# aouyang1/go-muse

Measured on AMD Instinct MI355X. Metric: series-pairs XCorr/sec at N=4096, 1M-series batch; achieved HBM GB/s, higher is better.
Workload: dtype f64

## Files before the change

### go-muse_amd/binding.py

```python
import ctypes
import os

import numpy as np

from . import build as _build

_i32 = ctypes.c_int32
_i64 = ctypes.c_int64
_f64 = ctypes.c_double
_vp = ctypes.c_void_p
_dp = ctypes.POINTER(ctypes.c_double)
_i32p = ctypes.POINTER(ctypes.c_int32)
_i64p = ctypes.POINTER(ctypes.c_int64)

MUSE_OK = 0
MUSE_ERR_INVALID = -1
MUSE_ERR_LENGTH = -2
MUSE_ERR_ZERO_STD = -3
MUSE_ERR_NO_DEVICE = -4
MUSE_ERR_HIP = -5
MUSE_ERR_UNSUPPORTED = -6
MUSE_ERR_NOMEM = -7
MUSE_ERR_EMPTY = -8
MUSE_LAG_WINDOW_MAX = 63
# ... 117 lines not shown
    "muse_test_many_lag_range_plan": (ctypes.c_int, [_i32, _i32, _i32, _i32, _i32, _i32p]),
    "muse_test_window_many_plan_rows": (ctypes.c_int, [_i32, _i32, _i32p, _i32p, _i32p, _i32p, _i32p, _i32p]),
    "muse_batch_run_many": (ctypes.c_int, [ctypes.POINTER(_vp), _i32, _i32p, _i32, _i32, _i32, _f64, _i32, _i32,
                                           _i64p, _i32p, _dp, _i32p, _dp]),
    "muse_batch_free": (ctypes.c_int, [_vp]),
    "muse_xcorr_with_x": (ctypes.c_int, [_vp, _dp, _dp, _i32, _i32, _dp, _i32p, _dp, _i32p]),
    "muse_xcorr": (ctypes.c_int, [_vp, _dp, _i32, _dp, _i32, _i32, _i32, _dp, _i32p, _dp, _i32p]),
    "muse_xcorr_groups": (ctypes.c_int, [_vp, _vp, _i32, _i32, _i32p, _dp, _i32p, _dp]),
    "muse_xcorr_batch": (ctypes.c_int, [_vp, _dp, _dp, _i64, _i32, _i32, _i32, _i32, _i32p, _dp, _i32p, _dp]),
    "muse_ctx_set_spectrum_cache": (ctypes.c_int, [_vp, _i32]),
    "muse_group_spectrum_cache": (ctypes.c_int, [_vp, _i64p, _i64p]),
    "muse_group_drop_spectrum_cache": (ctypes.c_int, [_vp]),
    "muse_test_spectrum_cache_limits": (ctypes.c_int, [_vp, _i64, _i64]),
    "muse_test_spectrum_cache_reader": (ctypes.c_int, [_vp, _i32]),
    "muse_test_spectrum_cache_policy": (ctypes.c_int, [_i64, _i32, _i32, _i32, _i64, _i64, _i64, _i32p, _i64p, _i64p]),
    "muse_test_batch_redo_pairs": (ctypes.c_int, [_vp, _i64p, _i64, _i64p]),
    "muse_next_pow2": (_i64, [_f64]),
}


class MuseError(RuntimeError):
    def __init__(self, status, message):
        super().__init__("muse_hip status %d: %s" % (status, message))
        self.status = status
        self.message = message


_lib = None


# ... 45 lines not shown
```

### go-muse_amd/csrc/capi_batch.hip

```cpp
#include "capi_internal.h"
#include "xcorr_huge.h"

using namespace muse;


int ilog2(int64_t n)
{
    int l = 0;
    while (((int64_t)1 << l) < n)
        l++;
    return l;
}

int build_spectrum(muse_ctx *ctx, const double *ref_host, int N, int n, int normalize, double x_scale,
                          double xc_scale, double2 *X, double2 *xc, float2 *xcf, double *xs, int *zero_std)
{
    double *dref = nullptr;
    int *dstat = nullptr;
    double2 *dscr = nullptr;
    HIP_TRY(dmalloc(ctx, &dref, (size_t)N * sizeof(double)));
    hipError_t e = dmalloc(ctx, &dstat, sizeof(int));
    if (e == hipSuccess && n > GENERIC_LDS_MAX_N)
        e = dmalloc(ctx, &dscr, (size_t)n * sizeof(double2));
    if (e == hipSuccess)
// ... 335 lines not shown
        kc.variant = KERNEL_REAL_SPLIT;
        kc.gsmall = ctx->gsmall[4];
    } else if ((b->n == 32768 || (b->n == 65536 && (b->N == b->n || b->c1))) && (ctx->variant == 0 || ctx->variant == 14) && !b->g->f32 && ctx->gsmall[4]) {
        kc.variant = KERNEL_REAL;
        kc.gsmall = ctx->gsmall[4];
    } else if (b->xcp && has_twl && (b->N == b->n || b->c1) && ((b->n >= 32768 && ctx->variant == 0) || (b->n >= 16384 && ctx->variant == 13))) {
        kc.variant = KERNEL_LONG;
    } else if (((b->n >= 512 && b->n <= 2048) || b->n == 8192 || b->n == 16384) && (ctx->variant == 0 || ctx->variant == 12)) {
        kc.variant = KERNEL_SMALL;
    } else if (((b->n >= 512 && b->n <= 2048) || b->n >= 8192) && (ctx->variant == 0 || ctx->variant == 11)) {
        kc.variant = KERNEL_STOCKHAM;
    }
    return kc;
}

int spectrum_cache_policy(int64_t rows, int32_t N, bool f32, int mode, int64_t min_rows, int64_t free_bytes, int64_t budget,
                          int64_t *rows_cached, int64_t *bytes)
{
    *rows_cached = 0;
    *bytes = 0;
    if (mode != 1 || f32 || N <= 2048 || N > 4096 || rows < std::max<int64_t>(min_rows, 2))
        return ZC_POLICY_NONE;
    const int64_t pairs = rows / 2;
    *rows_cached = 2 * pairs;
    *bytes = pairs * ZC_PAIR_BYTES;
    const int64_t limit = budget >= 0 ? budget : free_bytes / 2;
    return *bytes <= limit ? ZC_POLICY_BUILD : ZC_POLICY_DECLINED;
}

void group_drop_spectrum_cache(muse_group *g)
// ... 141 lines not shown
    ctx->zc_reader.store(reader);
    return MUSE_OK;
}

extern "C" int muse_test_spectrum_cache_policy(int64_t rows, int32_t N, int32_t f32, int32_t mode, int64_t min_rows,
                                               int64_t free_bytes, int64_t budget_bytes, int32_t *decision,
                                               int64_t *rows_cached, int64_t *bytes)
{
    if (!decision || !rows_cached || !bytes)
        return fail(MUSE_ERR_INVALID, "NULL output");
    *decision = spectrum_cache_policy(rows, N, f32 != 0, mode, min_rows < 0 ? ZC_MIN_ROWS : min_rows, free_bytes,
                                      budget_bytes < 0 ? -1 : budget_bytes, rows_cached, bytes);
    return MUSE_OK;
}

extern "C" int muse_test_batch_redo_pairs(muse_batch *b, int64_t *pairs, int64_t cap, int64_t *count)
{
    if (!b || !count || cap < 0 || (cap > 0 && !pairs))
        return fail(MUSE_ERR_INVALID, "bad redo-list arguments");
    *count = 0;
    int rc = use_device(b->ctx);
    if (rc)
        return rc;
    HIP_TRY(hipStreamSynchronize(b->stream()));
    if (!b->ovf_count || !b->ovf_list.p)
        return MUSE_OK;
    int listed = 0;
    HIP_TRY(hipMemcpy(&listed, b->ovf_count, sizeof(int), hipMemcpyDeviceToHost));
    *count = listed;
    const int64_t k = std::min<int64_t>(std::min<int64_t>(listed, cap), b->ovf_list.cap);
// ... 11 lines not shown
{
    *variant = -1;
    if (win_L < 0 && b->windowed())
        return MUSE_OK;
    if (b->n > GENERIC_MAX_N)
        return b->g->f32 ? fail(MUSE_ERR_UNSUPPORTED, "float32-storage groups run on the default kernels only (FFT lengths 512 ... 16384)") : MUSE_OK;
    const KernelChoice kc = choose_kernel(b, (b->g->M + 1) / 2);
    if (kc.error)
        return fail(MUSE_ERR_UNSUPPORTED, "%s", kc.error);
    if (win_L >= 0 && (!(kc.variant == KERNEL_R16_FOLD || kc.variant == KERNEL_R16_OCC3 || (kc.variant == KERNEL_SMALL && b->logn <= 11)) || 2 * win_L > b->n))
        return fail(MUSE_ERR_UNSUPPORTED, "the masked transform pass runs on the default kernels of FFT lengths 512 ... 4096");
    *variant = kc.variant;
    return MUSE_OK;
}

int batch_score(muse_batch *b, bool allow_spectrum_cache, int win_L, const SlideFuse *slide, int win_lneg)
{
    if (!b)
        return fail(MUSE_ERR_INVALID, "NULL batch");
    muse_ctx *ctx = b->ctx;
    int rc = use_device(ctx);
    if (rc)
        return rc;
    rc = group_ready(b->g, b->stream());
    if (rc)
        return rc;
    const int64_t M = b->g->M;
    if (M == 0)
        return MUSE_OK;
    const hipStream_t st = b->stream();
    rc = ensure_scores(b);
    if (rc)
        return rc;
    b->origin = ScoreOrigin{};
    if (win_L < 0 && b->windowed()) {
        b->scores_exact = true;
        return score_windowed(b);
    }
    if (b->n > GENERIC_MAX_N) {
        if (b->g->f32)
            return fail(MUSE_ERR_UNSUPPORTED, "float32-storage groups run on the default kernels only (FFT lengths 512 ... 16384)");
        b->scores_exact = true;
        return huge_score(b);
    }
    std::unique_lock<std::mutex> scratch_lock(ctx->stage_mu, std::defer_lock);
    if (b->n >= GENERIC_LDS_MAX_N)
        scratch_lock.lock();
    FusedParams p = base_params(b);
    b->scores_exact = true;
// ... 15 lines not shown
            b->origin = ScoreOrigin::in_window(MUSE_IN_WINDOW_MASKED, win_L, variant);
            set_window(p, win_L);
        }
    }
    if (slide) {
        if (variant != KERNEL_R16_FOLD || allow_spectrum_cache)
            return fail(MUSE_ERR_INVALID, "the fused slide runs in the default n = 4096 kernel, off the rows");
        p.slide_tails = slide->tails;
        p.slide_k = slide->k;
    }
    if (variant == KERNEL_GENERIC && b->n <= GENERIC_LDS_MAX_N)
        p.gscratch = nullptr;
    LaunchTimer timer(ctx, false, st);
    LaunchTimer redo_timer(ctx, true, st);
    if (variant == KERNEL_R16_FOLD) {
        HIP_TRY(b->ovf_list.ensure(ctx, 2 * p.npairs, st));
        p.ovf_count = b->ovf_count;
        p.work_counter = b->ovf_count + 1;
        p.ovf_list = b->ovf_list.p;
        HIP_TRY(hipMemsetAsync(b->ovf_count, 0, 2 * sizeof(int), st));
        ZcPlan plan;
        std::unique_lock<std::mutex> zc_lock(b->g->ready_mu, std::defer_lock);
        if (allow_spectrum_cache && win_L < 0 && spectrum_cache_candidate(b, variant)) {
            zc_lock.lock();
            rc = plan_spectrum_cache(b, plan);
            if (rc)
                return rc;
            if (!plan.use)
                zc_lock.unlock();
        }
        HIP_TRY(timer.begin());
        if (plan.use) {
            bool launched = false;
            const auto next_launch = [&]() {
                const hipError_t e = launched ? hipMemsetAsync(b->ovf_count + 1, 0, sizeof(int), st) : hipSuccess;
// ... 15 lines not shown
                                                               plan.tail_zpairs ? plan.tail_seg.zstat() : nullptr,
                                                               plan.tail_pair0, plan.tail_zpairs}, ctx->num_cus, st));
            }
            zc_lock.unlock();
        } else {
            HIP_TRY(launch_fused(p, variant, ctx->num_cus, st));
        }
        HIP_TRY(timer.end());
        FusedParams q = p;
        q.slide_tails = nullptr;
        q.slide_k = 0;
        q.pair_list = b->ovf_list.p;
        q.pair_count = b->ovf_count;
        q.dense_total = ctx->variant == 0 ? p.npairs : 0;
        q.npairs = std::min<long long>(p.npairs, (long long)ctx->num_cus * 3);
        HIP_TRY(redo_timer.begin());
        HIP_TRY(launch_fused(q, KERNEL_R16_OCC3, ctx->num_cus, st));
        HIP_TRY(redo_timer.end());
        if (p.npairs >= 1024 && !(b->handoff_host && b->handoff_M == M && b->handoff_rewrites == b->g->rewrites)) {
            if (!b->handoff_host)
                HIP_TRY(hmalloc(ctx, &b->handoff_host, sizeof(int)));
            *b->handoff_host = 0;
            b->handoff_M = M;
            b->handoff_rewrites = b->g->rewrites;
            HIP_TRY(hipMemcpyAsync(b->handoff_host, b->ovf_count, sizeof(int), hipMemcpyDeviceToHost, st));
        }
    } else if (variant == KERNEL_LONG) {
        HIP_TRY(b->ovf_list.ensure(ctx, 2 * p.npairs, st));
        p.ovf_count = b->ovf_count;
        p.ovf_list = b->ovf_list.p;
        HIP_TRY(hipMemsetAsync(b->ovf_count, 0, 2 * sizeof(int), st));
        HIP_TRY(timer.begin());
        HIP_TRY(launch_fused(p, variant, ctx->num_cus, st));
// ... 152 lines not shown
```

### go-muse_amd/csrc/capi_internal.h

```cpp
#pragma once
#include <hip/hip_runtime.h>

#include <algorithm>
#include <atomic>
#include <mutex>
#include <cmath>
#include <cstdarg>
#include <cstdio>
#include <cstdlib>
#include <cstring>
#include <ctime>
#include <limits>
#include <map>
#include <new>
#include <string>
#include <unordered_map>
#include <utility>
#include <vector>

#include "muse_hip.h"
#include "muse_hip_test.h"
#include "xcorr_kernels.h"

using namespace muse;
// ... 92 lines not shown
    MemPool dev_pool, host_pool;
    HugeWork huge;
    int huge_batch_mb = 0;
    std::mutex huge_mu;
    std::mutex small_mu;
    std::vector<std::pair<unsigned char *, int>> small_free;
    unsigned long long small_token = 0;
    std::mutex timing_mu;
    std::atomic<bool> rows_always_copy{false};
    std::vector<void *> rows_slots;
    std::mutex rows_mu;
    std::atomic<int> zc_mode{1};
    std::atomic<int64_t> zc_min_rows{ZC_MIN_ROWS};
    std::atomic<int64_t> zc_budget{-1};
    std::atomic<int> zc_reader{0};
    std::atomic<int> win_rows_slices{0};
    std::atomic<bool> in_window_force{false};
    std::atomic<int> slide_in_window_force{0};
    std::atomic<bool> gather_nt{false};
    std::atomic<int> refs{1};
};

struct muse_group {
    std::atomic<int> refs{1};
    muse_ctx *ctx = nullptr;
    double *rows = nullptr;
    float *rows32 = nullptr;
    bool f32 = false;
    size_t elem() const { return f32 ? sizeof(float) : sizeof(double); }
    void *base() const { return f32 ? (void *)rows32 : (void *)rows; }
// ... 76 lines not shown

struct muse_batch {
    muse_ctx *ctx = nullptr;
    muse_group *g = nullptr;
    hipStream_t own_stream = nullptr;
    hipStream_t stream() const { return own_stream ? own_stream : ctx->stream; }
    int32_t N = 0, n = 0, logn = 0;
    muse_spectrum *sp = nullptr;
    double *c1 = nullptr;
    double2 *X = nullptr, *xc = nullptr;
    double2 *xcp = nullptr;
    double2 *xcw = nullptr;
    float2 *xcf = nullptr;
    double *xs = nullptr;
    int *ovf_count = nullptr;
    int *handoff_host = nullptr;
    int64_t handoff_M = -1;
    uint64_t handoff_rewrites = 0;
    PoolBuf<long long> ovf_list;
    PoolBuf<double> mv;
    PoolBuf<int> lag;
    unsigned char *small_out = nullptr;
    int small_cap = 0;
    PoolBuf<int> gid_dev;
    std::vector<int32_t> gid_host;
    bool gid_valid = false;
    PoolBuf<unsigned long long> gkey;
    PoolBuf<long long> gfirst, gwin;
    GroupWork gw() const { return GroupWork{gkey.p, gfirst.p, gwin.p}; }
    PoolBuf<muse_record> rec;
// ... 99 lines not shown
void huge_free(muse_ctx *ctx);
int huge_reference(muse_ctx *ctx, const double *ref_host, int N, int n, double2 *X, double2 *table, int *zero_std);
int huge_score(muse_batch *b);
int huge_pairs(muse_ctx *ctx, const double *xrows, int64_t xstride, int Nx, int normalize_x, double x_scale, const double *yrows,
               int64_t ystride, int Ny, int normalize_y, int64_t M, int n, double cc_scale, double *mv, int *lag, int *nil, double *cc);
void adopt_spectrum(muse_batch *b);
int build_spectrum(muse_ctx *ctx, const double *ref_host, int N, int n, int normalize, double x_scale,
                          double xc_scale, double2 *X, double2 *xc, float2 *xcf, double *xs, int *zero_std);
hipError_t ensure_gscratch(muse_ctx *ctx, int64_t n, int slices_per_cu = muse::GSCRATCH_SLICES_PER_CU);
hipError_t ensure_twl(muse_ctx *ctx, int64_t n);
int ensure_scores(muse_batch *b);
struct SlideFuse {
    const void *tails;
    int32_t k;
};
int batch_score(muse_batch *b, bool allow_spectrum_cache, int win_L = -1, const SlideFuse *slide = nullptr, int win_lneg = -1);
int batch_score_check(muse_batch *b, int win_L, int *variant);
enum { ZC_POLICY_NONE = 0, ZC_POLICY_BUILD = 1, ZC_POLICY_DECLINED = 2 };
int spectrum_cache_policy(int64_t rows, int32_t N, bool f32, int mode, int64_t min_rows, int64_t free_bytes, int64_t budget,
                          int64_t *rows_cached, int64_t *bytes);
void group_drop_spectrum_cache(muse_group *g);
int score_windowed(muse_batch *b);
int check_window_request(const muse_batch *b, int32_t max_lag, bool f32);
int window_tables(muse_batch *b, int L, PoolBuf<double> &e, PoolBuf<double> &pw, int32_t *cached_L, hipStream_t st);
inline int32_t window_range_key(int origin, int W) { return 0x10000 + origin * 256 + W; }
struct LagRange {
    int hi, lneg;
    int W() const { return hi + lneg + 1; }
};
inline LagRange clip_lag_range(int64_t n, int32_t lag_lo, int32_t lag_hi)
{
// ... 7 lines not shown
{
    p.win = 1;
    p.win_lpos = L;
    p.win_lneg = window_lneg(L, p.n);
}
inline void set_window(muse::FusedParams &p, int lpos, int lneg)
{
    p.win = 1;
    p.win_lpos = lpos;
    p.win_lneg = lneg;
}
int check_own_window(const muse_batch *b, int32_t max_lag, int r = -1);
muse::FusedParams base_params(muse_batch *b);
int ensure_select_ws(muse_batch *b, int64_t M, int64_t G, bool with_gid, int K, bool on_device);
inline bool select_on_device(int32_t top_n, int64_t G) { return top_n <= TOPN_DEVICE_MAX && G > EXACT_FEED_MAX_GROUPS; }
muse_batch::RunKey run_key(const muse_batch *b, const int32_t *group_id, int64_t G, int32_t max_lag, int32_t top_n,
                                  double threshold, int32_t sign_filter, int32_t abs_scores);
int32_t screen_path(const muse_batch *b, const muse_batch::RunKey &key, bool already_scored);
int score_screened(muse_batch *b, int32_t max_lag, int32_t top_n, double threshold, int32_t sign_filter,
                          int32_t abs_scores, const int *gid_dev = nullptr, int64_t G = 0);
int upload_group_ids(muse_batch *b, const int32_t *group_id, int64_t M);
bool screen_guard_tripped(muse_batch *b);
int run_select(muse_batch *b, const int32_t *group_id, int32_t G_in, int64_t series_offset, int32_t max_lag,
                      int32_t top_n, double threshold, int32_t sign_filter, int32_t abs_scores,
                      std::vector<muse_record> &out, bool already_scored = false, bool prescreened = false);
void emit(const std::vector<muse_record> &sel, int64_t *out_series, int32_t *out_lag, double *out_score,
                 int32_t *out_count, double *out_mean_abs);
int check_select_args(const int32_t *group_id, int32_t G, int32_t sign_filter);
int upload_many_tab(muse_ctx *ctx, std::vector<void *> &tab, bool zscratch);
int check_batch_list(muse_batch *const *bs, int32_t R);
// ... 10 lines not shown
```

### go-muse_amd/csrc/capi_many.hip

```cpp
#include "capi_internal.h"

using namespace muse;


int upload_many_tab(muse_ctx *ctx, std::vector<void *> &tab, bool zscratch)
{
    if (zscratch)
        HIP_TRY(ctx->zscratch.ensure(ctx, (int64_t)ctx->num_cus * 4 * 4096, ctx->stream));
    HIP_TRY(ctx->many_tab.ensure(ctx, (int64_t)tab.size(), ctx->stream));
    HIP_TRY(hipStreamSynchronize(ctx->stream));
    ctx->many_host.swap(tab);
    HIP_TRY(hipMemcpyAsync(ctx->many_tab.p, ctx->many_host.data(), ctx->many_host.size() * sizeof(void *),
                           hipMemcpyHostToDevice, ctx->stream));
    return MUSE_OK;
}

extern "C" int muse_batch_read_scores(muse_batch *b, int32_t *lag, double *mv)
{
    if (!b)
        return fail(MUSE_ERR_INVALID, "NULL batch");
    int rc = use_device(b->ctx);
    if (rc)
        return rc;
    const int64_t M = b->g->M;
// ... 97 lines not shown
    if (range)
        set_window(p, win_L, win_lneg);
    else if (masked)
        set_window(p, win_L);
    HIP_TRY(b0->ovf_list.ensure(ctx, 2 * p.npairs, b0->stream()));
    p.ovf_count = b0->ovf_count;
    p.work_counter = b0->ovf_count + 1;
    p.ovf_list = b0->ovf_list.p;
    std::unique_lock<std::mutex> scratch_lock(ctx->stage_mu, std::defer_lock);
    if (long_n || real_n) {
        scratch_lock.lock();
        p.gscratch = ctx->gscratch.p;
        p.gscratch_slices = (long long)(ctx->gscratch.cap / b0->n);
    }
    LaunchTimer timer(ctx);
    HIP_TRY(hipMemsetAsync(b0->ovf_count, 0, 2 * sizeof(int), ctx->stream));
    HIP_TRY(timer.begin());
    if (small_n) {
        HIP_TRY(launch_fused_small(p, ctx->num_cus, ctx->stream));
    } else if (real_n) {
        p.gsmall = ctx->gsmall[4];
        HIP_TRY(launch_fused_real_split(p, ctx->num_cus, ctx->stream));
    } else if (long_n)
        HIP_TRY(launch_fused_long(p, ctx->num_cus, ctx->stream));
    else
        HIP_TRY(launch_fused_multi(p, ctx->num_cus, ctx->stream));
    HIP_TRY(timer.end());
    const bool redo = !small_n && !real_n;
    LaunchTimer redo_timer(ctx, true);
    if (redo)
// ... 89 lines not shown
```

### go-muse_amd/csrc/capi_run.hip

```cpp
#include "capi_internal.h"

using namespace muse;


namespace {
struct GoHeap {
    std::vector<muse_record> h;
    static bool less(const muse_record &a, const muse_record &b) { return std::fabs(a.score) < std::fabs(b.score); }
    void up(size_t j)
    {
        for (;;) {
            if (j == 0)
                break;
            size_t i = (j - 1) / 2;
            if (!less(h[j], h[i]))
                break;
            std::swap(h[i], h[j]);
            j = i;
        }
    }
    void down(size_t i0, size_t n)
    {
        size_t i = i0;
        for (;;) {
// ... 15 lines not shown
        up(h.size() - 1);
    }
    muse_record pop()
    {
        size_t n = h.size() - 1;
        std::swap(h[0], h[n]);
        down(0, n);
        muse_record r = h.back();
        h.pop_back();
        return r;
    }
};

std::vector<muse_record> heap_select(std::vector<muse_record> cands, int64_t top_n)
{
    std::stable_sort(cands.begin(), cands.end(), [](const muse_record &a, const muse_record &b) {
        if (a.group != b.group)
            return a.group < b.group;
        return a.series < b.series;
    });
    GoHeap hp;
    if (top_n > 0) {
        for (const auto &r : cands) {
            if ((int64_t)hp.h.size() == top_n) {
                if (std::fabs(r.score) > std::fabs(hp.h[0].score)) {
                    hp.pop();
                    hp.push(r);
                }
            } else {
                hp.push(r);
// ... 107 lines not shown
{
    unsigned long long token;
    int rc = small_acquire(b, sp.G, &token);
    if (rc)
        return rc;
    const volatile SmallSlot *slots = (const volatile SmallSlot *)b->small_out;
    HIP_TRY(launch_small_groups(sp, (SmallSlot *)b->small_out, token, b->stream()));
    StampWait wait(b);
    for (int g = sp.G - 1; g >= 0; g--)
        if ((rc = wait(&slots[g].stamp, token)))
            return rc;
    __atomic_thread_fence(__ATOMIC_ACQUIRE);
    *out = (const SmallSlot *)b->small_out;
    return MUSE_OK;
}
static bool direct_topn(int64_t G, int K)
{
    const int64_t nb = (G + TOPN_CHUNK - 1) / TOPN_CHUNK;
    return K >= 1 && K <= TOPN_DEVICE_MAX && nb * K + (nb + 1) / 2 <= SMALL_DIRECT_MAX_SLOTS;
}
static int direct_topn_reduce(muse_batch *b, const SelectParams &sp, int K, std::vector<muse_record> &cands)
{
    const int64_t nb = ((int64_t)sp.G + TOPN_CHUNK - 1) / TOPN_CHUNK;
    unsigned long long token;
    int rc = small_acquire(b, nb * K + (nb + 1) / 2, &token);
    if (rc)
        return rc;
    SmallSlot *cand = (SmallSlot *)b->small_out;
    CountSlot *cnt = (CountSlot *)(cand + nb * K);
    HIP_TRY(launch_topn_ungrouped(sp, K, cand, cnt, token, b->stream()));
    StampWait wait(b);
    for (int64_t blk = 0; blk < nb; blk++) {
        const volatile CountSlot *c = cnt + blk;
        if ((rc = wait(&c->stamp, token)))
            return rc;
        __atomic_thread_fence(__ATOMIC_ACQUIRE);
        const int n = (int)c->count;
        for (int r = 0; r < n; r++) {
            const volatile SmallSlot *sl = cand + blk * K + r;
            if ((rc = wait(&sl->stamp, token)))
                return rc;
            __atomic_thread_fence(__ATOMIC_ACQUIRE);
            cands.push_back(muse_record{sl->series, sl->score, sl->lag, (int32_t)std::min<int64_t>(sl->series, 0x7fffffffLL)});
        }
    }
    return MUSE_OK;
}

int check_select_args(const int32_t *group_id, int32_t G, int32_t sign_filter)
{
    if (sign_filter < -1 || sign_filter > 1)
        return fail(MUSE_ERR_INVALID, "sign_filter must be -1, 0 or 1");
// ... 4 lines not shown

int run_select(muse_batch *b, const int32_t *group_id, int32_t G_in, int64_t series_offset, int32_t max_lag,
                      int32_t top_n, double threshold, int32_t sign_filter, int32_t abs_scores,
                      std::vector<muse_record> &out, bool already_scored, bool prescreened)
{
    out.clear();
    muse_ctx *ctx = b->ctx;
    const int64_t M = b->g->M;
    int rc = check_select_args(group_id, G_in, sign_filter);
    if (rc)
        return rc;
    const muse_batch::RunKey rkey = run_key(b, group_id, group_id ? (int64_t)G_in : 0, max_lag, top_n, threshold, sign_filter, abs_scores);
    const int32_t path = prescreened ? MUSE_RUN_PATH_SCREENED : screen_path(b, rkey, already_scored);
    const bool screened = path == MUSE_RUN_PATH_SCREENED;
    b->last_path = path;
    rc = (already_scored || screened) ? MUSE_OK : muse_batch_score(b);
    if (rc)
        return rc;
    const int64_t G = group_id ? (int64_t)G_in : M;
    if (M == 0 || G == 0 || top_n <= 0)
        return MUSE_OK;
    if (G > 0x7fffffffLL)
        return fail(MUSE_ERR_UNSUPPORTED, "more than 2^31-1 groups on one device");
    const bool on_device = select_on_device(top_n, G);
    const int K = on_device ? top_n : 1;
    const bool small = !on_device && !screened && small_run(M, G, group_id != nullptr);
    const bool direct = on_device && !screened && !group_id && direct_topn(G, K);
    rc = ensure_select_ws(b, M, small || direct ? 0 : G, group_id != nullptr, K, on_device && !direct);
    if (rc)
        return rc;
    rc = upload_group_ids(b, group_id, M);
// ... 15 lines not shown
    sp.max_lag = max_lag;
    sp.threshold = threshold;
    sp.sign_filter = sign_filter;
    sp.series_offset = series_offset;
    sp.include = screened ? b->include.p : nullptr;
    std::vector<muse_record> cands;
    if (small) {
        const SmallSlot *slot;
        rc = small_reduce(b, sp, &slot);
        if (rc)
            return rc;
        for (int64_t g = 0; g < G; g++)
            if (slot[g].key != 0u)
                cands.push_back(muse_record{slot[g].series, slot[g].score, slot[g].lag, (int32_t)g});
    } else if (direct) {
        rc = direct_topn_reduce(b, sp, K, cands);
        if (rc)
            return rc;
    } else if (on_device) {
        HIP_TRY(launch_group_reduce(sp, b->gw(), b->rec.p, b->selkey.p, b->stream()));
        const int64_t nb = (G + TOPN_CHUNK - 1) / TOPN_CHUNK;
        HIP_TRY(launch_topn(b->rec.p, b->selkey.p, (int)G, K, b->cand.p, b->cnt.p, b->stream()));
        const int *cnt = b->cnt_host.p;
        const muse_record *cand = b->cand_host.p;
        HIP_TRY(hipMemcpyAsync(b->cnt_host.p, b->cnt.p, (size_t)nb * sizeof(int), hipMemcpyDeviceToHost, b->stream()));
        HIP_TRY(hipMemcpyAsync(b->cand_host.p, b->cand.p, (size_t)(nb * K) * sizeof(muse_record), hipMemcpyDeviceToHost,
                               b->stream()));
        HIP_TRY(hipStreamSynchronize(b->stream()));
        for (int64_t blk = 0; blk < nb; blk++)
            for (int r = 0; r < cnt[(size_t)blk]; r++)
                cands.push_back(cand[(size_t)(blk * K + r)]);
        if (screened && (int64_t)*b->refine_host * 4 > (M + 1) / 2)
            b->costly_key = rkey;
// ... 204 lines not shown
```

### go-muse_amd/csrc/capi_screen.hip

```cpp
#include "capi_internal.h"

using namespace muse;


muse_batch::RunKey run_key(const muse_batch *b, const int32_t *group_id, int64_t G, int32_t max_lag, int32_t top_n,
                                  double threshold, int32_t sign_filter, int32_t abs_scores)
{
    muse_batch::RunKey k;
    k.M = b->g->M;
    k.G = group_id ? G : 0;
    k.grouped = group_id ? 1 : 0;
    k.max_lag = max_lag;
    k.top_n = top_n;
    k.threshold = threshold;
    k.sign_filter = sign_filter;
    k.abs_scores = abs_scores ? 1 : 0;
    return k;
}

int32_t screen_path(const muse_batch *b, const muse_batch::RunKey &key, bool already_scored)
{
    const muse_ctx *ctx = b->ctx;
    const int64_t M = b->g->M;
    const bool length_ok = b->n >= 512 && b->n <= 65536;
// ... 62 lines not shown
    HIP_TRY(b->est_save.ensure(ctx, 4 * npairs, st));
    HIP_TRY(b->ovf_list.ensure(ctx, 2 * npairs, st));
    if (b->sp->xmax < 0.0) {
        std::vector<double2> X((size_t)(b->n / 2 + 1));
        HIP_TRY(hipMemcpyAsync(X.data(), b->X, X.size() * sizeof(double2), hipMemcpyDeviceToHost, ctx->stream));
        HIP_TRY(hipStreamSynchronize(ctx->stream));
        double m = 0.0;
        for (const double2 &x : X)
            m = std::max(m, std::hypot(x.x, x.y));
        b->sp->xmax = m;
    }
    plan.Es = screen_error_scaled(b->sp->xmax, b->n) * ctx->screen_e_scale;
    HIP_TRY(hipMemsetAsync(b->err_dev, 0, sizeof(unsigned long long), ctx->stream));
    HIP_TRY(hipMemsetAsync(b->scr_flags.p, 0, (size_t)M * sizeof(unsigned), ctx->stream));
    HIP_TRY(hipMemsetAsync(b->include.p, 0, (size_t)M, ctx->stream));
    HIP_TRY(hipMemsetAsync(b->ovf_count, 0, 2 * sizeof(int), ctx->stream));
    return MUSE_OK;
}

static FusedParams screen_pass_params(muse_batch *b, int32_t max_lag, const ScreenPlan &plan, bool need_sign = true)
{
    FusedParams p = base_params(b);
    p.scr_need_sign = need_sign ? 1 : 0;
    p.scr_flags = b->scr_flags.p;
    p.scr_var = b->scr_var.p;
    p.scr_max_lag = max_lag;
    p.screen_delta = 2.0 * plan.Es;
    return p;
}

// ... 223 lines not shown
```

### go-muse_amd/csrc/reduce_kernels.hip

```cpp
#include <hip/hip_runtime.h>
#include <stdint.h>

#include "xcorr_kernels.h"

namespace muse {

constexpr long long IDX_NONE = 0x7fffffffffffffffLL;

__device__ __forceinline__ double clamp_score(double mv, int abs_scores)
{
    if (abs_scores) {
        double v = fabs(mv);
        if (v > 1.0)
            v = 1.0;
        return v;
    }
    double v = mv;
    if (v > 1.0)
        v = 1.0;
    else if (v < -1.0)
        v = -1.0;
    return v;
}
__device__ __forceinline__ unsigned long long abs_bits(double v)
// ... 225 lines not shown
#pragma unroll
    for (int o = 32; o > 0; o >>= 1) {
        const unsigned long long u = __shfl_xor(v, o, 64);
        v = u > v ? u : v;
    }
    return v;
}
__device__ __forceinline__ int wave_min_i32(int v)
{
#pragma unroll
    for (int o = 32; o > 0; o >>= 1)
        v = min(v, __shfl_xor(v, o, 64));
    return v;
}

__global__ __launch_bounds__(256) void topn_kernel(const muse_record *__restrict__ rec,
                                                   const unsigned long long *__restrict__ selkey, int G, int K,
                                                   muse_record *cand, int *cnt)
{
    __shared__ unsigned long long sk[4];
    __shared__ int si[4];
    const int t = threadIdx.x, lane = t & 63, wave = t >> 6;
    const int base = blockIdx.x * TOPN_CHUNK;
    unsigned long long k[16];
#pragma unroll
    for (int m = 0; m < 16; m++) {
        const int g = base + t + 256 * m;
        k[m] = g < G ? selkey[g] : 0ull;
    }
    int r = 0;
    for (; r < K; r++) {
        unsigned long long bk = 0ull;
        int bm = 0;
#pragma unroll
        for (int m = 0; m < 16; m++)
            if (k[m] > bk) {
                bk = k[m];
                bm = m;
            }
        const unsigned long long wk = wave_max_u64(bk);
        if (lane == 0)
            sk[wave] = wk;
        __syncthreads();
        unsigned long long BK = sk[0];
        BK = sk[1] > BK ? sk[1] : BK;
        BK = sk[2] > BK ? sk[2] : BK;
        BK = sk[3] > BK ? sk[3] : BK;
        if (BK == 0ull)
            break;
        int ci = (bk == BK) ? (t + 256 * bm) : 0x7fffffff;
        ci = wave_min_i32(ci);
        if (lane == 0)
            si[wave] = ci;
        __syncthreads();
        const int CI = min(min(si[0], si[1]), min(si[2], si[3]));
        if (t == (CI & 255)) {
            const int mm = CI >> 8;
#pragma unroll
            for (int m = 0; m < 16; m++)
                if (m == mm)
                    k[m] = 0ull;
            cand[(long long)blockIdx.x * K + r] = rec[base + CI];
        }
        __syncthreads();
    }
    if (t == 0)
        cnt[blockIdx.x] = r;
}


__global__ __launch_bounds__(256) void topn_ungrouped_kernel(SelectParams sp, int K, SmallSlot *cand, CountSlot *cnt,
                                                             unsigned long long token)
{
    __shared__ unsigned long long sk[4];
    __shared__ int si[4];
    __shared__ int picked[TOPN_DEVICE_MAX];
    const int t = threadIdx.x, lane = t & 63, wave = t >> 6;
    const long long base = (long long)blockIdx.x * TOPN_CHUNK;
    unsigned long long k[16];
#pragma unroll
    for (int m = 0; m < 16; m++) {
        const long long g = base + t + 256 * m;
        k[m] = 0ull;
        if (g < sp.G) {
            const double s = clamp_score(sp.mv[g], sp.abs_scores);
            if (passed(s, sp.lag[g], sp))
                k[m] = abs_bits(s) + 1ull;
        }
    }
    int r = 0;
    for (; r < K; r++) {
        unsigned long long bk = 0ull;
        int bm = 0;
#pragma unroll
        for (int m = 0; m < 16; m++)
            if (k[m] > bk) {
                bk = k[m];
                bm = m;
            }
        const unsigned long long wk = wave_max_u64(bk);
        if (lane == 0)
            sk[wave] = wk;
        __syncthreads();
        unsigned long long BK = sk[0];
        BK = sk[1] > BK ? sk[1] : BK;
        BK = sk[2] > BK ? sk[2] : BK;
        BK = sk[3] > BK ? sk[3] : BK;
        if (BK == 0ull)
            break;
        int ci = (bk == BK) ? (t + 256 * bm) : 0x7fffffff;
        ci = wave_min_i32(ci);
        if (lane == 0)
            si[wave] = ci;
        __syncthreads();
        const int CI = min(min(si[0], si[1]), min(si[2], si[3]));
        if (t == (CI & 255)) {
            const int mm = CI >> 8;
#pragma unroll
            for (int m = 0; m < 16; m++)
                if (m == mm)
                    k[m] = 0ull;
            picked[r] = CI;
        }
        __syncthreads();
    }
    __syncthreads();
    for (int i = t; i < r; i += 256) {
        const long long g = base + picked[i];
        muse_record rec;
        rec.series = g + sp.series_offset;
        rec.score = clamp_score(sp.mv[g], sp.abs_scores);
        rec.lag = sp.lag[g];
        rec.group = 0;
        write_slot(cand + (long long)blockIdx.x * K + i, rec, 1ull, token);
    }
    if (t == 0) {
        cnt[blockIdx.x].count = (unsigned long long)r;
        asm volatile("s_waitcnt vmcnt(0)" ::: "memory");
        cnt[blockIdx.x].stamp = token;
        asm volatile("" ::: "memory");
    }
}

hipError_t launch_topn_ungrouped(const SelectParams &sp, int K, SmallSlot *cand, CountSlot *cnt, unsigned long long token,
                                 hipStream_t stream)
{
    if (sp.G <= 0 || sp.group_id || sp.include || K < 1 || K > TOPN_DEVICE_MAX)
        return hipErrorInvalidValue;
    const int nb = (sp.G + TOPN_CHUNK - 1) / TOPN_CHUNK;
    hipLaunchKernelGGL(topn_ungrouped_kernel, dim3(nb), dim3(256), 0, stream, sp, K, cand, cnt, token);
    return hipGetLastError();
}

struct RowBounds {
    bool nan;
    double lo, hi;
    bool pass_may, pass_must;
};
__device__ __forceinline__ RowBounds row_bounds(double sv, double var, unsigned f, const ScreenSelect &q)
{
    RowBounds r;
    r.nan = (f & SCR_NAN) != 0u;
    if (r.nan || (f & SCR_REFINE)) {
        r.lo = 0.0;
        r.hi = 1.0;
// ... 406 lines not shown
```

### go-muse_amd/csrc/xcorr_kernels.h

```cpp
#pragma once
#include <hip/hip_runtime.h>
#include <stdint.h>
#include <type_traits>

#include "muse_hip.h"

namespace muse {

enum { KERNEL_GENERIC = 0, KERNEL_R16_OCC3 = 6, KERNEL_STOCKHAM = 10, KERNEL_R16_FOLD = 11, KERNEL_SMALL = 12, KERNEL_LONG = 13, KERNEL_REAL = 14, KERNEL_REAL_SPLIT = 15 };

struct FusedParams {
    const double *rows;
    const float *rows32;
    long long M;
    long long stride;
    long long npairs;
    int N;
    int n;
    int logn;
    int normalize_y;
    const double2 *xc;
    const double2 *tw1;
    const double2 *tw2;
    const double2 *xcp;
// ... 249 lines not shown
struct SmallSlot {
    long long series;
    double score;
    int lag;
    unsigned key;
    unsigned long long stamp;
};
static_assert(sizeof(SmallSlot) == 32, "one slot = one 32-byte block");
hipError_t launch_small_groups(const SelectParams &sp, SmallSlot *out, unsigned long long token, hipStream_t stream);
constexpr int SMALL_DIRECT_MAX_SLOTS = 131072;
struct CountSlot {
    unsigned long long count;
    unsigned long long stamp;
};
hipError_t launch_topn_ungrouped(const SelectParams &sp, int K, SmallSlot *cand, CountSlot *cnt, unsigned long long token,
                                 hipStream_t stream);
struct SingleGroupOut {
    muse_record rec;
    unsigned long long state;
};
hipError_t launch_single_group(const double *mv, const int *lag, long long M, int abs_scores, long long series_offset,
                               SingleGroupOut *out, hipStream_t stream);
hipError_t launch_topn(const muse_record *rec, const unsigned long long *selkey, int G, int K, muse_record *cand,
                       int *cnt, hipStream_t stream);

}
```

### go-muse_amd/muse.py

```python
import ctypes
import math
import sys
import threading
import uuid
import weakref

import numpy as np

from . import binding as B
from .binding import MuseError

DefaultLabel = "uid"

SignFilter_POS = 1
SignFilter_NEG = -1
SignFilter_ANY = 0


class Engine:

    def __init__(self, device=0):
        self._h = ctypes.c_void_p()
        B.check(B.load().muse_ctx_create(int(device), ctypes.byref(self._h)))
        self.device = int(device)
# ... 33 lines not shown

    def set_screening(self, enable, min_rows=None):
        B.check(B.load().muse_ctx_set_screening(self._h, (int(min_rows) if min_rows and min_rows > 1 else 1) if enable else 0))

    def set_screen_bound_scale(self, scale):
        B.check(B.load().muse_test_set_screen_bound_scale(self._h, float(scale)))

    def set_spectrum_cache(self, on):
        B.check(B.load().muse_ctx_set_spectrum_cache(self._h, 1 if on else 0))

    def spectrum_cache_limits(self, min_rows=-1, budget_bytes=-1):
        B.check(B.load().muse_test_spectrum_cache_limits(self._h, int(min_rows), int(budget_bytes)))

    def spectrum_cache_reader(self, reader=0):
        B.check(B.load().muse_test_spectrum_cache_reader(self._h, int(reader)))

    def trim(self):
        B.check(B.load().muse_ctx_trim(self._h))

    def pool_stats(self):
        v = [ctypes.c_int64(0) for _ in range(4)]
        B.check(B.load().muse_test_pool_stats(self._h, *[ctypes.byref(x) for x in v]))
        return tuple(int(x.value) for x in v)

    def xcorr_repeat(self, repeat):
        B.check(B.load().muse_test_xcorr_repeat(self._h, int(repeat)))

    def huge_batch_mb(self, megabytes):
        B.check(B.load().muse_test_huge_batch_mb(self._h, int(megabytes)))

# ... 1435 lines not shown
```

Before: 165.2 million.

## Defer redo launch and counter reset into top-n kernel for empty overflow lists

Adds a run-tail policy for ungrouped, unscreened fold-pass runs. When the host already knows the overflow list was empty, the policy skips both the counter memset and the redo kernel launch. The top-n kernel then reads and clears the counters, and a redo plus a second top-n pass run only if entries turn up. The top-n selection is rewritten as a per-thread bitonic sort followed by DPP wave reductions and a rank merge across waves, which replaces the K iterations of block-wide barriers. A partial-selection fast path is also added to host heap_select. This adds complexity and a fallback path that rescans when the list turns out not to be empty.

```diff
diff --git a/go-muse_amd/binding.py b/go-muse_amd/binding.py
--- a/go-muse_amd/binding.py
+++ b/go-muse_amd/binding.py
@@ -155,6 +155,8 @@
     "muse_test_spectrum_cache_limits": (ctypes.c_int, [_vp, _i64, _i64]),
     "muse_test_spectrum_cache_reader": (ctypes.c_int, [_vp, _i32]),
     "muse_test_spectrum_cache_policy": (ctypes.c_int, [_i64, _i32, _i32, _i32, _i64, _i64, _i64, _i32p, _i64p, _i64p]),
+    "muse_test_run_tail": (ctypes.c_int, [_vp, _i32]),
+    "muse_test_run_tail_policy": (ctypes.c_int, [_i64, _i32, _i32, _i32, _i32, _i32, _i32, _i64, _i64, _i64, _i64, _i32, _i32, _i32p]),
     "muse_test_batch_redo_pairs": (ctypes.c_int, [_vp, _i64p, _i64, _i64p]),
     "muse_next_pow2": (_i64, [_f64]),
 }
diff --git a/go-muse_amd/csrc/capi_batch.hip b/go-muse_amd/csrc/capi_batch.hip
--- a/go-muse_amd/csrc/capi_batch.hip
+++ b/go-muse_amd/csrc/capi_batch.hip
@@ -373,6 +373,20 @@
     return kc;
 }
 
+int run_tail_policy(const RunTailFacts &f)
+{
+    if (!f.fold_pass || f.windowed || f.grouped || f.screened)
+        return RUN_TAIL_FULL;
+    if (f.M <= 0 || !select_on_device(f.top_n, f.M) || !direct_topn(f.M, f.top_n))
+        return RUN_TAIL_FULL;
+    bool empty = f.count_known && f.count == 0 && f.count_M == f.M && f.count_rewrites == f.rewrites;
+    if (f.force >= 0)
+        empty = f.force == 1;
+    if (!empty)
+        return RUN_TAIL_FULL;
+    return f.counters_zero ? RUN_TAIL_FAST : RUN_TAIL_PREPARE;
+}
+
 int spectrum_cache_policy(int64_t rows, int32_t N, bool f32, int mode, int64_t min_rows, int64_t free_bytes, int64_t budget,
                           int64_t *rows_cached, int64_t *bytes)
 {
@@ -544,6 +558,40 @@
     return MUSE_OK;
 }
 
+extern "C" int muse_test_run_tail(muse_ctx *ctx, int32_t belief)
+{
+    if (!ctx)
+        return fail(MUSE_ERR_INVALID, "NULL context");
+    if (belief < -1 || belief > 1)
+        return fail(MUSE_ERR_INVALID, "run tail belief %d (-1 = what the host knows, 0 = the list is never empty, 1 = it is empty)", (int)belief);
+    ctx->run_tail_force.store(belief);
+    return MUSE_OK;
+}
+
+extern "C" int muse_test_run_tail_policy(int64_t M, int32_t top_n, int32_t grouped, int32_t screened, int32_t windowed, int32_t fold_pass,
+                                         int32_t count_known, int64_t count, int64_t count_M, int64_t count_rewrites, int64_t rewrites,
+                                         int32_t counters_zero, int32_t belief, int32_t *step)
+{
+    if (!step)
+        return fail(MUSE_ERR_INVALID, "NULL output");
+    RunTailFacts f;
+    f.M = M;
+    f.top_n = top_n;
+    f.grouped = grouped != 0;
+    f.screened = screened != 0;
+    f.windowed = windowed != 0;
+    f.fold_pass = fold_pass != 0;
+    f.count_known = count_known != 0;
+    f.count = count;
+    f.count_M = count_M;
+    f.count_rewrites = (uint64_t)count_rewrites;
+    f.rewrites = (uint64_t)rewrites;
+    f.counters_zero = counters_zero != 0;
+    f.force = belief;
+    *step = run_tail_policy(f);
+    return MUSE_OK;
+}
+
 extern "C" int muse_test_batch_redo_pairs(muse_batch *b, int64_t *pairs, int64_t cap, int64_t *count)
 {
     if (!b || !count || cap < 0 || (cap > 0 && !pairs))
@@ -585,7 +633,16 @@
     return MUSE_OK;
 }
 
-int batch_score(muse_batch *b, bool allow_spectrum_cache, int win_L, const SlideFuse *slide, int win_lneg)
+int batch_redo(muse_batch *b, const FusedParams &q)
+{
+    LaunchTimer redo_timer(b->ctx, true, b->stream());
+    HIP_TRY(redo_timer.begin());
+    HIP_TRY(launch_fused(q, KERNEL_R16_OCC3, b->ctx->num_cus, b->stream()));
+    HIP_TRY(redo_timer.end());
+    return MUSE_OK;
+}
+
+int batch_score(muse_batch *b, bool allow_spectrum_cache, int win_L, const SlideFuse *slide, int win_lneg, RunTail *tail)
 {
     if (!b)
         return fail(MUSE_ERR_INVALID, "NULL batch");
@@ -604,6 +661,8 @@
     if (rc)
         return rc;
     b->origin = ScoreOrigin{};
+    const bool counters_were_zero = b->counters_zero;
+    b->counters_zero = false;
     if (win_L < 0 && b->windowed()) {
         b->scores_exact = true;
         return score_windowed(b);
@@ -649,11 +708,29 @@
     LaunchTimer timer(ctx, false, st);
     LaunchTimer redo_timer(ctx, true, st);
     if (variant == KERNEL_R16_FOLD) {
+        int tail_mode = RUN_TAIL_FULL;
+        if (tail) {
+            RunTailFacts f;
+            f.M = M;
+            f.top_n = tail->top_n;
+            f.grouped = tail->grouped;
+            f.screened = tail->screened;
+            f.fold_pass = win_L < 0 && !slide;
+            f.count_known = b->handoff_host != nullptr;
+            f.count = f.count_known ? *(volatile int *)b->handoff_host : 0;
+            f.count_M = b->handoff_M;
+            f.count_rewrites = b->handoff_rewrites;
+            f.rewrites = b->g->rewrites;
+            f.counters_zero = counters_were_zero;
+            f.force = ctx->run_tail_force.load();
+            tail->mode = tail_mode = run_tail_policy(f);
+        }
         HIP_TRY(b->ovf_list.ensure(ctx, 2 * p.npairs, st));
         p.ovf_count = b->ovf_count;
         p.work_counter = b->ovf_count + 1;
         p.ovf_list = b->ovf_list.p;
-        HIP_TRY(hipMemsetAsync(b->ovf_count, 0, 2 * sizeof(int), st));
+        if (tail_mode != RUN_TAIL_FAST)
+            HIP_TRY(hipMemsetAsync(b->ovf_count, 0, 2 * sizeof(int), st));
         ZcPlan plan;
         std::unique_lock<std::mutex> zc_lock(b->g->ready_mu, std::defer_lock);
         if (allow_spectrum_cache && win_L < 0 && spectrum_cache_candidate(b, variant)) {
@@ -699,9 +776,13 @@
         q.pair_count = b->ovf_count;
         q.dense_total = ctx->variant == 0 ? p.npairs : 0;
         q.npairs = std::min<long long>(p.npairs, (long long)ctx->num_cus * 3);
-        HIP_TRY(redo_timer.begin());
-        HIP_TRY(launch_fused(q, KERNEL_R16_OCC3, ctx->num_cus, st));
-        HIP_TRY(redo_timer.end());
+        if (tail_mode == RUN_TAIL_FAST) {
+            tail->redo = q;
+        } else {
+            HIP_TRY(redo_timer.begin());
+            HIP_TRY(launch_fused(q, KERNEL_R16_OCC3, ctx->num_cus, st));
+            HIP_TRY(redo_timer.end());
+        }
         if (p.npairs >= 1024 && !(b->handoff_host && b->handoff_M == M && b->handoff_rewrites == b->g->rewrites)) {
             if (!b->handoff_host)
                 HIP_TRY(hmalloc(ctx, &b->handoff_host, sizeof(int)));
diff --git a/go-muse_amd/csrc/capi_internal.h b/go-muse_amd/csrc/capi_internal.h
--- a/go-muse_amd/csrc/capi_internal.h
+++ b/go-muse_amd/csrc/capi_internal.h
@@ -130,6 +130,7 @@
     std::atomic<int64_t> zc_min_rows{ZC_MIN_ROWS};
     std::atomic<int64_t> zc_budget{-1};
     std::atomic<int> zc_reader{0};
+    std::atomic<int> run_tail_force{-1};
     std::atomic<int> win_rows_slices{0};
     std::atomic<bool> in_window_force{false};
     std::atomic<int> slide_in_window_force{0};
@@ -236,6 +237,7 @@
     float2 *xcf = nullptr;
     double *xs = nullptr;
     int *ovf_count = nullptr;
+    bool counters_zero = false;
     int *handoff_host = nullptr;
     int64_t handoff_M = -1;
     uint64_t handoff_rewrites = 0;
@@ -365,7 +367,28 @@
     const void *tails;
     int32_t k;
 };
-int batch_score(muse_batch *b, bool allow_spectrum_cache, int win_L = -1, const SlideFuse *slide = nullptr, int win_lneg = -1);
+struct RunTail {
+    bool grouped = false, screened = false;
+    int32_t top_n = 0;
+    int mode = 0;
+    muse::FusedParams redo{};
+};
+int batch_score(muse_batch *b, bool allow_spectrum_cache, int win_L = -1, const SlideFuse *slide = nullptr, int win_lneg = -1,
+                RunTail *tail = nullptr);
+int batch_redo(muse_batch *b, const muse::FusedParams &q);
+enum { RUN_TAIL_FULL = 0, RUN_TAIL_PREPARE = 1, RUN_TAIL_FAST = 2 };
+struct RunTailFacts {
+    int64_t M = 0;
+    int32_t top_n = 0;
+    bool grouped = false, screened = false, windowed = false;
+    bool fold_pass = false;
+    bool count_known = false;
+    int64_t count = 0, count_M = -1;
+    uint64_t count_rewrites = 0, rewrites = 0;
+    bool counters_zero = false;
+    int force = -1;
+};
+int run_tail_policy(const RunTailFacts &f);
 int batch_score_check(muse_batch *b, int win_L, int *variant);
 enum { ZC_POLICY_NONE = 0, ZC_POLICY_BUILD = 1, ZC_POLICY_DECLINED = 2 };
 int spectrum_cache_policy(int64_t rows, int32_t N, bool f32, int mode, int64_t min_rows, int64_t free_bytes, int64_t budget,
@@ -403,6 +426,11 @@
 muse::FusedParams base_params(muse_batch *b);
 int ensure_select_ws(muse_batch *b, int64_t M, int64_t G, bool with_gid, int K, bool on_device);
 inline bool select_on_device(int32_t top_n, int64_t G) { return top_n <= TOPN_DEVICE_MAX && G > EXACT_FEED_MAX_GROUPS; }
+inline bool direct_topn(int64_t G, int K)
+{
+    const int64_t nb = (G + TOPN_CHUNK - 1) / TOPN_CHUNK;
+    return K >= 1 && K <= TOPN_DEVICE_MAX && nb * K + (nb + 1) / 2 <= SMALL_DIRECT_MAX_SLOTS;
+}
 muse_batch::RunKey run_key(const muse_batch *b, const int32_t *group_id, int64_t G, int32_t max_lag, int32_t top_n,
                                   double threshold, int32_t sign_filter, int32_t abs_scores);
 int32_t screen_path(const muse_batch *b, const muse_batch::RunKey &key, bool already_scored);
diff --git a/go-muse_amd/csrc/capi_many.hip b/go-muse_amd/csrc/capi_many.hip
--- a/go-muse_amd/csrc/capi_many.hip
+++ b/go-muse_amd/csrc/capi_many.hip
@@ -135,6 +135,7 @@
         p.gscratch_slices = (long long)(ctx->gscratch.cap / b0->n);
     }
     LaunchTimer timer(ctx);
+    b0->counters_zero = false;
     HIP_TRY(hipMemsetAsync(b0->ovf_count, 0, 2 * sizeof(int), ctx->stream));
     HIP_TRY(timer.begin());
     if (small_n) {
diff --git a/go-muse_amd/csrc/capi_run.hip b/go-muse_amd/csrc/capi_run.hip
--- a/go-muse_amd/csrc/capi_run.hip
+++ b/go-muse_amd/csrc/capi_run.hip
@@ -53,6 +53,32 @@
 
 std::vector<muse_record> heap_select(std::vector<muse_record> cands, int64_t top_n)
 {
+    if (top_n > 0 && cands.size() > 1) {
+        const size_t k = (size_t)std::min<int64_t>((int64_t)cands.size(), top_n + 1);
+        std::vector<std::pair<double, size_t>> top;
+        top.reserve(k + 1);
+        bool plain = true;
+        for (size_t i = 0; plain && i < cands.size(); i++) {
+            const double v = std::fabs(cands[i].score);
+            plain = v == v;
+            if (top.size() == k && !(v > top.back().first))
+                continue;
+            size_t at = top.size();
+            while (at > 0 && top[at - 1].first < v)
+                at--;
+            top.insert(top.begin() + (long)at, std::make_pair(v, i));
+            if (top.size() > k)
+                top.pop_back();
+        }
+        for (size_t i = 1; plain && i < top.size(); i++)
+            plain = top[i - 1].first > top[i].first;
+        if (plain) {
+            std::vector<muse_record> out((size_t)std::min<int64_t>((int64_t)cands.size(), top_n));
+            for (size_t i = 0; i < out.size(); i++)
+                out[i] = cands[top[i].second];
+            return out;
+        }
+    }
     std::stable_sort(cands.begin(), cands.end(), [](const muse_record &a, const muse_record &b) {
         if (a.group != b.group)
             return a.group < b.group;
@@ -190,12 +216,8 @@
     *out = (const SmallSlot *)b->small_out;
     return MUSE_OK;
 }
-static bool direct_topn(int64_t G, int K)
-{
-    const int64_t nb = (G + TOPN_CHUNK - 1) / TOPN_CHUNK;
-    return K >= 1 && K <= TOPN_DEVICE_MAX && nb * K + (nb + 1) / 2 <= SMALL_DIRECT_MAX_SLOTS;
-}
-static int direct_topn_reduce(muse_batch *b, const SelectParams &sp, int K, std::vector<muse_record> &cands)
+static int direct_topn_reduce(muse_batch *b, const SelectParams &sp, int K, std::vector<muse_record> &cands, int *counters = nullptr,
+                              bool clear_listed = false, int64_t *listed = nullptr)
 {
     const int64_t nb = ((int64_t)sp.G + TOPN_CHUNK - 1) / TOPN_CHUNK;
     unsigned long long token;
@@ -204,14 +226,18 @@
         return rc;
     SmallSlot *cand = (SmallSlot *)b->small_out;
     CountSlot *cnt = (CountSlot *)(cand + nb * K);
-    HIP_TRY(launch_topn_ungrouped(sp, K, cand, cnt, token, b->stream()));
+    HIP_TRY(launch_topn_ungrouped(sp, K, cand, cnt, token, b->stream(), counters, clear_listed));
     StampWait wait(b);
+    cands.reserve((size_t)(nb * K));
     for (int64_t blk = 0; blk < nb; blk++) {
         const volatile CountSlot *c = cnt + blk;
         if ((rc = wait(&c->stamp, token)))
             return rc;
         __atomic_thread_fence(__ATOMIC_ACQUIRE);
-        const int n = (int)c->count;
+        const unsigned long long count = c->count;
+        const int n = (int)(count & 0xffffffffull);
+        if (blk == 0 && listed)
+            *listed = (int64_t)(count >> 32);
         for (int r = 0; r < n; r++) {
             const volatile SmallSlot *sl = cand + blk * K + r;
             if ((rc = wait(&sl->stamp, token)))
@@ -246,7 +272,11 @@
     const int32_t path = prescreened ? MUSE_RUN_PATH_SCREENED : screen_path(b, rkey, already_scored);
     const bool screened = path == MUSE_RUN_PATH_SCREENED;
     b->last_path = path;
-    rc = (already_scored || screened) ? MUSE_OK : muse_batch_score(b);
+    RunTail tail;
+    tail.grouped = group_id != nullptr;
+    tail.screened = screened;
+    tail.top_n = top_n;
+    rc = (already_scored || screened) ? MUSE_OK : batch_score(b, true, -1, nullptr, -1, &tail);
     if (rc)
         return rc;
     const int64_t G = group_id ? (int64_t)G_in : M;
@@ -292,9 +322,23 @@
             if (slot[g].key != 0u)
                 cands.push_back(muse_record{slot[g].series, slot[g].score, slot[g].lag, (int32_t)g});
     } else if (direct) {
-        rc = direct_topn_reduce(b, sp, K, cands);
+        int64_t listed = 0;
+        rc = direct_topn_reduce(b, sp, K, cands, tail.mode != RUN_TAIL_FULL ? b->ovf_count : nullptr, tail.mode == RUN_TAIL_PREPARE, &listed);
         if (rc)
             return rc;
+        if (tail.mode == RUN_TAIL_FAST && listed != 0) {
+            if (b->handoff_host && b->handoff_M == M && b->handoff_rewrites == b->g->rewrites)
+                *b->handoff_host = (int)listed;
+            rc = batch_redo(b, tail.redo);
+            if (rc)
+                return rc;
+            cands.clear();
+            rc = direct_topn_reduce(b, sp, K, cands);
+            if (rc)
+                return rc;
+        } else if (tail.mode != RUN_TAIL_FULL) {
+            b->counters_zero = tail.mode == RUN_TAIL_PREPARE || listed == 0;
+        }
     } else if (on_device) {
         HIP_TRY(launch_group_reduce(sp, b->gw(), b->rec.p, b->selkey.p, b->stream()));
         const int64_t nb = (G + TOPN_CHUNK - 1) / TOPN_CHUNK;
diff --git a/go-muse_amd/csrc/capi_screen.hip b/go-muse_amd/csrc/capi_screen.hip
--- a/go-muse_amd/csrc/capi_screen.hip
+++ b/go-muse_amd/csrc/capi_screen.hip
@@ -100,6 +100,7 @@
     HIP_TRY(hipMemsetAsync(b->err_dev, 0, sizeof(unsigned long long), ctx->stream));
     HIP_TRY(hipMemsetAsync(b->scr_flags.p, 0, (size_t)M * sizeof(unsigned), ctx->stream));
     HIP_TRY(hipMemsetAsync(b->include.p, 0, (size_t)M, ctx->stream));
+    b->counters_zero = false;
     HIP_TRY(hipMemsetAsync(b->ovf_count, 0, 2 * sizeof(int), ctx->stream));
     return MUSE_OK;
 }
diff --git a/go-muse_amd/csrc/reduce_kernels.hip b/go-muse_amd/csrc/reduce_kernels.hip
--- a/go-muse_amd/csrc/reduce_kernels.hip
+++ b/go-muse_amd/csrc/reduce_kernels.hip
@@ -263,13 +263,117 @@
     return v;
 }
 
+__device__ __forceinline__ bool beats(unsigned long long ka, int ia, unsigned long long kb, int ib)
+{
+    return ka > kb || (ka == kb && ia < ib);
+}
+template <int CTRL, int ROW_MASK> __device__ __forceinline__ void dpp_best(unsigned long long &k, int &i)
+{
+    const int ulo = __builtin_amdgcn_update_dpp(0, (int)(unsigned)k, CTRL, ROW_MASK, 0xf, false);
+    const int uhi = __builtin_amdgcn_update_dpp(0, (int)(unsigned)(k >> 32), CTRL, ROW_MASK, 0xf, false);
+    const int ui = __builtin_amdgcn_update_dpp(0x7fffffff, i, CTRL, ROW_MASK, 0xf, false);
+    const unsigned long long uk = ((unsigned long long)(unsigned)uhi << 32) | (unsigned long long)(unsigned)ulo;
+    if (beats(uk, ui, k, i)) {
+        k = uk;
+        i = ui;
+    }
+}
+__device__ __forceinline__ int chunk_topk(unsigned long long (&k)[16], int K, int *picked)
+{
+    __shared__ unsigned long long ck[4][TOPN_DEVICE_MAX];
+    __shared__ int ci[4][TOPN_DEVICE_MAX];
+    __shared__ int cw[4];
+    const int t = threadIdx.x, lane = t & 63, wave = t >> 6;
+    int mi[16];
+#pragma unroll
+    for (int m = 0; m < 16; m++)
+        mi[m] = m;
+#pragma unroll
+    for (int p = 1; p < 16; p <<= 1)
+#pragma unroll
+        for (int q = p; q >= 1; q >>= 1)
+#pragma unroll
+            for (int j = q % p; j + q < 16; j += 2 * q)
+#pragma unroll
+                for (int i = 0; i < q; i++) {
+                    const int a = i + j, b = i + j + q;
+                    if (b < 16 && a / (2 * p) == b / (2 * p) && beats(k[b], mi[b], k[a], mi[a])) {
+                        const unsigned long long tk = k[a];
+                        k[a] = k[b];
+                        k[b] = tk;
+                        const int tm = mi[a];
+                        mi[a] = mi[b];
+                        mi[b] = tm;
+                    }
+                }
+    unsigned long long ms = 0ull;
+#pragma unroll
+    for (int m = 0; m < 16; m++)
+        ms |= (unsigned long long)mi[m] << (4 * m);
+    int r = 0;
+    for (; r < K; r++) {
+        unsigned long long bk = k[0];
+        const int mine = bk != 0ull ? t + 256 * (int)(ms & 15ull) : 0x7fffffff;
+        int bi = mine;
+        dpp_best<0x111, 0xf>(bk, bi);
+        dpp_best<0x112, 0xf>(bk, bi);
+        dpp_best<0x114, 0xf>(bk, bi);
+        dpp_best<0x118, 0xf>(bk, bi);
+        dpp_best<0x142, 0xa>(bk, bi);
+        dpp_best<0x143, 0xc>(bk, bi);
+        const unsigned long long BK = ((unsigned long long)(unsigned)__builtin_amdgcn_readlane((int)(unsigned)(bk >> 32), 63) << 32) |
+                                      (unsigned long long)(unsigned)__builtin_amdgcn_readlane((int)(unsigned)bk, 63);
+        const int BI = __builtin_amdgcn_readlane(bi, 63);
+        if (BK == 0ull)
+            break;
+        if (lane == 0) {
+            ck[wave][r] = BK;
+            ci[wave][r] = BI;
+        }
+        if (mine == BI) {
+#pragma unroll
+            for (int m = 0; m < 15; m++)
+                k[m] = k[m + 1];
+            k[15] = 0ull;
+            ms >>= 4;
+        }
+    }
+    if (lane == 0)
+        cw[wave] = r;
+    __syncthreads();
+    const int c0 = cw[0], c1 = c0 + cw[1], c2 = c1 + cw[2], total = c2 + cw[3];
+    for (int c = t; c < total; c += 256) {
+        const int w = (c >= c0) + (c >= c1) + (c >= c2);
+        const int pos = c - (w == 0 ? 0 : w == 1 ? c0 : w == 2 ? c1 : c2);
+        const unsigned long long xk = ck[w][pos];
+        const int xi = ci[w][pos];
+        int rank = pos;
+        for (int w2 = 0; w2 < 4; w2++) {
+            if (w2 == w)
+                continue;
+            int lo = 0, hi = cw[w2];
+            while (lo < hi) {
+                const int mid = (lo + hi) >> 1;
+                if (beats(ck[w2][mid], ci[w2][mid], xk, xi))
+                    lo = mid + 1;
+                else
+                    hi = mid;
+            }
+            rank += lo;
+        }
+        if (rank < K)
+            picked[rank] = xi;
+    }
+    __syncthreads();
+    return total < K ? total : K;
+}
+
 __global__ __launch_bounds__(256) void topn_kernel(const muse_record *__restrict__ rec,
                                                    const unsigned long long *__restrict__ selkey, int G, int K,
                                                    muse_record *cand, int *cnt)
 {
-    __shared__ unsigned long long sk[4];
-    __shared__ int si[4];
-    const int t = threadIdx.x, lane = t & 63, wave = t >> 6;
+    __shared__ int picked[TOPN_DEVICE_MAX];
+    const int t = threadIdx.x;
     const int base = blockIdx.x * TOPN_CHUNK;
     unsigned long long k[16];
 #pragma unroll
@@ -277,54 +381,19 @@
         const int g = base + t + 256 * m;
         k[m] = g < G ? selkey[g] : 0ull;
     }
-    int r = 0;
-    for (; r < K; r++) {
-        unsigned long long bk = 0ull;
-        int bm = 0;
-#pragma unroll
-        for (int m = 0; m < 16; m++)
-            if (k[m] > bk) {
-                bk = k[m];
-                bm = m;
-            }
-        const unsigned long long wk = wave_max_u64(bk);
-        if (lane == 0)
-            sk[wave] = wk;
-        __syncthreads();
-        unsigned long long BK = sk[0];
-        BK = sk[1] > BK ? sk[1] : BK;
-        BK = sk[2] > BK ? sk[2] : BK;
-        BK = sk[3] > BK ? sk[3] : BK;
-        if (BK == 0ull)
-            break;
-        int ci = (bk == BK) ? (t + 256 * bm) : 0x7fffffff;
-        ci = wave_min_i32(ci);
-        if (lane == 0)
-            si[wave] = ci;
-        __syncthreads();
-        const int CI = min(min(si[0], si[1]), min(si[2], si[3]));
-        if (t == (CI & 255)) {
-            const int mm = CI >> 8;
-#pragma unroll
-            for (int m = 0; m < 16; m++)
-                if (m == mm)
-                    k[m] = 0ull;
-            cand[(long long)blockIdx.x * K + r] = rec[base + CI];
-        }
-        __syncthreads();
-    }
+    const int r = chunk_topk(k, K, picked);
+    for (int i = t; i < r; i += 256)
+        cand[(long long)blockIdx.x * K + i] = rec[base + picked[i]];
     if (t == 0)
         cnt[blockIdx.x] = r;
 }
 
 
 __global__ __launch_bounds__(256) void topn_ungrouped_kernel(SelectParams sp, int K, SmallSlot *cand, CountSlot *cnt,
-                                                             unsigned long long token)
-{
-    __shared__ unsigned long long sk[4];
-    __shared__ int si[4];
+                                                             unsigned long long token, int *counters, int clear_listed)
+{
     __shared__ int picked[TOPN_DEVICE_MAX];
-    const int t = threadIdx.x, lane = t & 63, wave = t >> 6;
+    const int t = threadIdx.x;
     const long long base = (long long)blockIdx.x * TOPN_CHUNK;
     unsigned long long k[16];
 #pragma unroll
@@ -337,43 +406,7 @@
                 k[m] = abs_bits(s) + 1ull;
         }
     }
-    int r = 0;
-    for (; r < K; r++) {
-        unsigned long long bk = 0ull;
-        int bm = 0;
-#pragma unroll
-        for (int m = 0; m < 16; m++)
-            if (k[m] > bk) {
-                bk = k[m];
-                bm = m;
-            }
-        const unsigned long long wk = wave_max_u64(bk);
-        if (lane == 0)
-            sk[wave] = wk;
-        __syncthreads();
-        unsigned long long BK = sk[0];
-        BK = sk[1] > BK ? sk[1] : BK;
-        BK = sk[2] > BK ? sk[2] : BK;
-        BK = sk[3] > BK ? sk[3] : BK;
-        if (BK == 0ull)
-            break;
-        int ci = (bk == BK) ? (t + 256 * bm) : 0x7fffffff;
-        ci = wave_min_i32(ci);
-        if (lane == 0)
-            si[wave] = ci;
-        __syncthreads();
-        const int CI = min(min(si[0], si[1]), min(si[2], si[3]));
-        if (t == (CI & 255)) {
-            const int mm = CI >> 8;
-#pragma unroll
-            for (int m = 0; m < 16; m++)
-                if (m == mm)
-                    k[m] = 0ull;
-            picked[r] = CI;
-        }
-        __syncthreads();
-    }
-    __syncthreads();
+    const int r = chunk_topk(k, K, picked);
     for (int i = t; i < r; i += 256) {
         const long long g = base + picked[i];
         muse_record rec;
@@ -384,7 +417,14 @@
         write_slot(cand + (long long)blockIdx.x * K + i, rec, 1ull, token);
     }
     if (t == 0) {
-        cnt[blockIdx.x].count = (unsigned long long)r;
+        unsigned long long listed = 0ull;
+        if (counters && blockIdx.x == 0) {
+            listed = (unsigned long long)(unsigned)counters[0];
+            counters[1] = 0;
+            if (clear_listed)
+                counters[0] = 0;
+        }
+        cnt[blockIdx.x].count = (unsigned long long)r | (listed << 32);
         asm volatile("s_waitcnt vmcnt(0)" ::: "memory");
         cnt[blockIdx.x].stamp = token;
         asm volatile("" ::: "memory");
@@ -392,12 +432,12 @@
 }
 
 hipError_t launch_topn_ungrouped(const SelectParams &sp, int K, SmallSlot *cand, CountSlot *cnt, unsigned long long token,
-                                 hipStream_t stream)
+                                 hipStream_t stream, int *counters, bool clear_listed)
 {
     if (sp.G <= 0 || sp.group_id || sp.include || K < 1 || K > TOPN_DEVICE_MAX)
         return hipErrorInvalidValue;
     const int nb = (sp.G + TOPN_CHUNK - 1) / TOPN_CHUNK;
-    hipLaunchKernelGGL(topn_ungrouped_kernel, dim3(nb), dim3(256), 0, stream, sp, K, cand, cnt, token);
+    hipLaunchKernelGGL(topn_ungrouped_kernel, dim3(nb), dim3(256), 0, stream, sp, K, cand, cnt, token, counters, clear_listed ? 1 : 0);
     return hipGetLastError();
 }
 
diff --git a/go-muse_amd/csrc/xcorr_kernels.h b/go-muse_amd/csrc/xcorr_kernels.h
--- a/go-muse_amd/csrc/xcorr_kernels.h
+++ b/go-muse_amd/csrc/xcorr_kernels.h
@@ -287,7 +287,7 @@
     unsigned long long stamp;
 };
 hipError_t launch_topn_ungrouped(const SelectParams &sp, int K, SmallSlot *cand, CountSlot *cnt, unsigned long long token,
-                                 hipStream_t stream);
+                                 hipStream_t stream, int *counters = nullptr, bool clear_listed = false);
 struct SingleGroupOut {
     muse_record rec;
     unsigned long long state;
diff --git a/go-muse_amd/muse.py b/go-muse_amd/muse.py
--- a/go-muse_amd/muse.py
+++ b/go-muse_amd/muse.py
@@ -71,6 +71,9 @@
 
     def spectrum_cache_reader(self, reader=0):
         B.check(B.load().muse_test_spectrum_cache_reader(self._h, int(reader)))
+
+    def run_tail(self, belief=-1):
+        B.check(B.load().muse_test_run_tail(self._h, int(belief)))
 
     def trim(self):
         B.check(B.load().muse_ctx_trim(self._h))
```

Result: no change. 165.7 million, median of 6 (+0.3%).
